# LahiruCooray/rl-aerial-manipulator

Hardware: AMD Instinct MI355X
Metric: env-steps/sec (whole node), hexacopter+arm waypoint task at 4096 envs/GPU (higher is better)
Workload: dtype f32

## Files before the change

rl-aerial-manipulator_amd/csrc/amenv_capi.hip:

```cpp
#include <hip/hip_runtime.h>
#include <hip/hip_ext.h>

#include <algorithm>
#include <cmath>
#include <cstdio>
#include <cstdlib>
#include <cstring>
#include <mutex>
#include <new>
#include <string>
#include <vector>

#include "amenv_kernels.hpp"
#include "amenv_team.hpp"
#include "amenv_team_host.hpp"
#include "amenv_quad.hpp"
#include "amenv_team_policy.hpp"
#include "amenv_quad_policy.hpp"
#include "amenv_lane_policy.hpp"
#include "amenv_rigid_policy.hpp"
#include "amenv_obsnorm.hpp"
#include "amenv_policy.hpp"
#include "amenv_train.hpp"
#include "amenv_mlp_train.hpp"
// ... 310 lines not shown
bool rigid_pol_ok(const amenv_config& c) { return c.vehicle.n_joints == 0 && c.dtype == AMENV_F32 && (c.vehicle.n_rotors == 4 || c.vehicle.n_rotors == 6); }
bool arm_pol_ok(const amenv_config& c) { return c.vehicle.n_joints == 3 && c.dtype == AMENV_F32; }

constexpr int kTeamAutoMax = 6144;
constexpr int kArmkAutoMax = 32768;

const char* select_step_family(const amenv_config& c, StepFamily* out) {
  const int want = c.step_kernel, n = c.num_envs;
  const bool autok = want == AMENV_KERNEL_AUTO, f32 = c.dtype == AMENV_F32, arm = zxx_arm1(c);
  StepFamily f = StepFamily::Lane;
  if (arm && (want == AMENV_KERNEL_TEAM || (f32 && autok && n <= kTeamAutoMax)))
    f = StepFamily::Team;
  else if (arm && c.task.rk4_substeps == 1 && (want == AMENV_KERNEL_STAGED || (f32 && autok && n > kTeamAutoMax && n <= kArmkAutoMax)))
    f = StepFamily::Staged;
  else if (arm && f32 && (want == AMENV_KERNEL_HELPER || (autok && n <= 65536)))
    f = StepFamily::TwoWave;
  else if (quad_ok(c) && want == AMENV_KERNEL_TEAM)
    f = StepFamily::Quad;
  else if (c.vehicle.n_joints == 0 && c.block_size == 0 && (autok ? n <= 32768 : want == AMENV_KERNEL_HELPER && n <= 64 * kStatsReplicas))
    f = StepFamily::LaneHelper;
  if (f == StepFamily::Lane && want == AMENV_KERNEL_HELPER)
    return "AMENV_KERNEL_HELPER is built for fp32 z,x,x-arm vehicles and for rigid vehicles with block_size = 0 "
           "and at most 65536 envs (its Monitor wave owns one of the 1024 replicas of the running totals per tile)";
  if (f == StepFamily::Lane && want == AMENV_KERNEL_TEAM)
    return "AMENV_KERNEL_TEAM is built for the 6-rotor vehicle with the z,x,x arm (16 lanes per env; fp64 = logic-gate build) and for "
           "fp32 rigid vehicles with 4 or 6 rotors, the single-waypoint v2 task and block_size = 0 (4 lanes per env)";
  if (f == StepFamily::Lane && want == AMENV_KERNEL_STAGED)
    return "AMENV_KERNEL_STAGED is built for the 6-rotor vehicle with the z,x,x arm (fp64 = logic-gate build), the single-waypoint v2 task "
           "and rk4_substeps = 1";
  *out = f;
  return nullptr;
}

std::string kernel_name(const amenv& e) {
  const amenv_config& c = e.cfg;
  const char* t = c.dtype == AMENV_F64 ? "double" : "float";
  const int nrot = (c.vehicle.n_rotors == 4 || c.vehicle.n_rotors == 6) ? c.vehicle.n_rotors : AMENV_MAX_ROTORS;
  const int kw = is_v1(&c) ? 2 : (c.task.num_waypoints == 1 ? 1 : AMENV_MAX_WAYPOINTS);
  char buf[200] = "";
  switch (e.family) {
    case StepFamily::Lane:
      std::snprintf(buf, sizeof(buf), "step_kernel<%s,NROT=%d,KW=%d,%s> block=%d", t, nrot, kw, c.vehicle.n_joints ? "v2+arm3" : (is_v1(&c) ? "v1" : "v2"), e.block); break;
    case StepFamily::LaneHelper:
      std::snprintf(buf, sizeof(buf), "step_kernel_pw<%s,NROT=%d,KW=%d,%s> (main wave + reset wave [+ observation wave + Monitor wave] per 64-env tile)", t, nrot, kw,
                    is_v1(&c) ? "v1" : "v2"); break;
    case StepFamily::Quad:
      std::snprintf(buf, sizeof(buf), "step_kernel_quad<NROT=%d,v2> (4 lanes per env, 16 envs per wave + episode-end helper wave)", c.vehicle.n_rotors); break;
    case StepFamily::Team:
      std::snprintf(buf, sizeof(buf), "step_kernel_team<%s,NROT=6,v2+arm3> (16 lanes per env: 4 RK4 stages x 4 components, 4 envs per wave + episode-end helper wave)", t); break;
    case StepFamily::Staged:
      std::snprintf(buf, sizeof(buf), "step_kernel_armk<%s,NROT=6> block=320 (4 RK4 stage waves + main wave per 64-env tile)", t); break;
    case StepFamily::TwoWave:
      std::snprintf(buf, sizeof(buf), "step_kernel_arm2w<float,NROT=6> block=128 (2 waves per 64-env tile)"); break;
  }
  std::string name = buf;
  if (e.dr) name += " +dr";
  if (e.pub_nj == 1 || e.pub_nj == 2) name += " [" + std::to_string(e.pub_nj) + "-joint arm: phantom links inside, pack / unpack at the C ABI]";
  return name;
}

template <typename... P, typename... A>
hipError_t launch(const amenv& e, bool timed, void (*k)(P...), dim3 grid, dim3 block, size_t lds, hipStream_t s, A... args) {
  if (timed) hipExtLaunchKernelGGL(k, grid, block, lds, s, e.ev_start, e.ev_stop, 0, args...);
  else hipLaunchKernelGGL(k, grid, block, lds, s, args...);
  return hipGetLastError();
}

template <typename T, int NROT, int KW, int VAR, int NJ, bool DR>
hipError_t launch_rollout(const amenv& e, const StepIO& io, int T_steps, hipStream_t s) {
  const StepTail tl{io.terminal_obs, io.ep_return, io.ep_len, io.stats};
  const ColdParams C = make_cold(e);
  const uint32_t tb = e.tile_bytes;
  const int32_t n = e.cfg.num_envs;
  switch (e.family) {
    case StepFamily::Team:
      if constexpr (NJ == 3 && sizeof(T) == 4 && !DR)
        return launch(e, false, rollout_kernel_team<NROT>, dim3(e.n_tiles * 16), dim3(64), 0, s, e.blob, tb, n, reinterpret_cast<const float*>(io.actions), io.obs,
                      static_cast<float*>(io.reward), io.done, io.info, T_steps, tl, C, make_team<T>(e));
      return hipErrorInvalidValue;
    case StepFamily::Quad:
      if constexpr (NJ == 0 && sizeof(T) == 4 && KW == 1 && VAR == VAR_V2 && (NROT == 4 || NROT == 6) && !DR)
        return launch(e, false, rollout_kernel_quad<NROT>, dim3(e.n_tiles * 4), dim3(64), 0, s, e.blob, tb, n, io.actions, io.obs, static_cast<float*>(io.reward), io.done,
                      io.info, T_steps, tl, C, make_quad(e));
      return hipErrorInvalidValue;
    case StepFamily::Lane: case StepFamily::LaneHelper: case StepFamily::Staged: case StepFamily::TwoWave:
      break;
  }
  ArmArg<T, NJ> AA;
  if constexpr (NJ > 0) AA.p = make_arm<T>(e); else AA.unused = 0;
  const int bs = e.block;
  return launch(e, false, rollout_kernel<T, NROT, KW, VAR, NJ, DR>, dim3((e.n_tiles * 64 + bs - 1) / bs), dim3(bs), size_t(bs) * ObsDim<VAR, NJ>::value * sizeof(float), s,
                e.blob, tb, n, io.actions, io.obs, io.reward, io.done, io.info, T_steps, tl, make_hot<T, NROT>(e), C, AA, make_dr<DR>(e));
}

template <typename T, int NROT, int KW, int VAR, int NJ = 0, bool DR = false>
hipError_t launch_step(const amenv& e, const StepIO& io, int T_steps, hipStream_t s, bool timed) {
  if (T_steps > 0) return launch_rollout<T, NROT, KW, VAR, NJ, DR>(e, io, T_steps, s);
  ArmArg<T, NJ> AA;
  if constexpr (NJ > 0) AA.p = make_arm<T>(e); else AA.unused = 0;
  const HotParams<T, NROT> P = make_hot<T, NROT>(e);
  const ColdParams C = make_cold(e);
  const StepTail tl{io.terminal_obs, io.ep_return, io.ep_len, io.stats};
  const uint32_t tb = e.tile_bytes;
  const int32_t n = e.cfg.num_envs;
  switch (e.family) {
    case StepFamily::Team:
      if constexpr (NJ == 3 && !DR) {
        const TeamParamsT<T> TP = make_team<T>(e);
        return launch(e, timed, step_kernel_team<T, NROT>, dim3(e.n_tiles * 16), dim3(128), 0, s, e.blob, n, int32_t(e.n_tiles * 16),
                      reinterpret_cast<const float*>(io.actions), TP.consts, io.obs, static_cast<T*>(io.reward), io.done, io.info, tl, C);
      }
      break;
    case StepFamily::Staged:
      if constexpr (NJ == 3 && !DR) {
        if constexpr (sizeof(T) == 8) {
          hipError_t ea = hipFuncSetAttribute(reinterpret_cast<const void*>(&step_kernel_armk<T, NROT>), hipFuncAttributeMaxDynamicSharedMemorySize, 96 * 1024);
          if (ea != hipSuccess) return ea;
        }
        const size_t lds = size_t(64 * ObsDim<VAR, NJ>::value + 12 * 64) * sizeof(float) + size_t((4 * kAggSlots + 6) * 64) * sizeof(T);
        return launch(e, timed, step_kernel_armk<T, NROT>, dim3(e.n_tiles), dim3(320), lds, s, e.blob, tb, n, io.actions, io.obs, io.reward, io.done, io.info, tl, P, C, AA);
      }
      break;
    case StepFamily::TwoWave:
      if constexpr (NJ == 3 && sizeof(T) == 4 && !DR) {
        const size_t lds = size_t(64 * ObsDim<VAR, NJ>::value + (kArmXchgSlots + 12) * 64) * sizeof(float);
        return launch(e, timed, step_kernel_arm2w<T, NROT>, dim3(e.n_tiles), dim3(128), lds, s, e.blob, tb, n, io.actions, io.obs, io.reward, io.done, io.info, tl, P, C, AA);
      }
      break;
    case StepFamily::Quad:
      if constexpr (NJ == 0 && sizeof(T) == 4 && KW == 1 && VAR == VAR_V2 && (NROT == 4 || NROT == 6) && !DR)
        return launch(e, timed, step_kernel_quad<NROT>, dim3(e.n_tiles * 4), dim3(128), 0, s, e.blob, tb, n, io.actions, io.obs, static_cast<float*>(io.reward), io.done,
                      io.info, tl, C, make_quad(e));
      break;
    case StepFamily::LaneHelper:
      if constexpr (NJ == 0) {
        const size_t lds = size_t(64 * ObsDim<VAR, 0>::value + 12 * 64) * sizeof(float);
        return launch(e, timed, step_kernel_pw<T, NROT, KW, VAR, DR>, dim3(e.n_tiles), dim3((KW == 1 && VAR == VAR_V2) ? 256 : 128), lds, s, e.blob, tb, n, io.actions,
                      io.obs, io.reward, io.done, io.info, tl, P, C, make_dr<DR>(e));
      }
      break;
    case StepFamily::Lane: {
      const int bs = e.block;
// ... 946 lines not shown
```

rl-aerial-manipulator_amd/csrc/amenv_team.hpp:

```cpp
#pragma once
#include "amenv_kernels.hpp"

#define AMENV_FN __device__ __forceinline__

namespace amenv_dev {

template <int CTRL> __device__ __forceinline__ float dpp_(float v) {
  return __builtin_bit_cast(float, __builtin_amdgcn_update_dpp(0, __builtin_bit_cast(int, v), CTRL, 0xF, 0xF, true));
}
template <int CTRL> __device__ __forceinline__ double dpp_(double v) {
  const int lo = __builtin_amdgcn_update_dpp(0, __double2loint(v), CTRL, 0xF, 0xF, true);
  const int hi = __builtin_amdgcn_update_dpp(0, __double2hiint(v), CTRL, 0xF, 0xF, true);
  return __hiloint2double(hi, lo);
}
template <int P0, int P1, int P2, int P3> __device__ __forceinline__ float qp(float v) { return dpp_<P0 | (P1 << 2) | (P2 << 4) | (P3 << 6)>(v); }
template <int P0, int P1, int P2, int P3> __device__ __forceinline__ double qp(double v) { return dpp_<P0 | (P1 << 2) | (P2 << 4) | (P3 << 6)>(v); }
template <int P0, int P1, int P2, int P3> __device__ __forceinline__ int qpi(int v) {
  return __builtin_amdgcn_update_dpp(0, v, P0 | (P1 << 2) | (P2 << 4) | (P3 << 6), 0xF, 0xF, true);
}
template <int N> __device__ __forceinline__ float row_ror(float v) { return dpp_<0x120 + N>(v); }
template <int N> __device__ __forceinline__ double row_ror(double v) { return dpp_<0x120 + N>(v); }
template <int N> __device__ __forceinline__ float row_shr(float v) { return dpp_<0x110 + N>(v); }
template <int N> __device__ __forceinline__ double row_shr(double v) { return dpp_<0x110 + N>(v); }
__device__ __forceinline__ float sel(bool m, float a, float b) { return m ? a : b; }
__device__ __forceinline__ double sel(bool m, double a, double b) { return m ? a : b; }
__device__ __forceinline__ int sel(bool m, int a, int b) { return m ? a : b; }
__device__ __forceinline__ void sincos_t(float x, float& s, float& c) { s = __sinf(x); c = __cosf(x); }
__device__ __forceinline__ void sincos_t(double x, double& s, double& c) { s = sin(x); c = cos(x); }
__device__ __forceinline__ float scale_action_f32(float a, float s1, float s2) { return (a * s1) * s2; }
__device__ __forceinline__ double scale_action_f32(double a, double s1, double s2) { return double((float(a) * float(s1)) * float(s2)); }
__device__ __forceinline__ float joint_cmd_f32(float a, float half, float mid) { return __builtin_fmaf(a, half, mid); }
__device__ __forceinline__ double joint_cmd_f32(double a, double half, double mid) { return double(__builtin_fmaf(float(a), float(half), float(mid))); }

}

#include "amenv_team_math.hpp"

namespace amenv_dev {

using TeamParams = TeamParamsT<float>;
using TeamState = TeamStateT<float>;

__device__ __forceinline__ int team_group_of_block(int b, int nblocks) { return (b & 7) * (nblocks >> 3) + (b >> 3); }

template <typename X>
struct TeamEnvT {
  TeamStateT<X> y;
  X WP;
  X final_yaw, last_distance, ep_return;
  int32_t step, counter, flags, episode;
};
using TeamEnv = TeamEnvT<float>;

template <typename X>
struct TeamLaneT {
  int lane, cc, bb;
  bool q0, q1, q2, lead;
  uint32_t offA, offB, offC;
  bool okA, okB, okC;
  X c[((kTeamConsts + 3) / 4) * 4];
  __device__ __forceinline__ void init(const TeamParamsT<X>& P) { init(P.consts); }
  __device__ __forceinline__ void init(const void* table) {
    lane = int(threadIdx.x) & 63; cc = lane & 3; bb = (lane >> 2) & 3;
    q0 = bb == 0; q1 = bb == 1; q2 = bb == 2; lead = (lane & 15) == 0;
    offA = uint32_t(cc + 3 * bb + (bb == 3 ? 1 : 0));
    offB = uint32_t(13 + 3 * bb - (bb == 3 ? 2 : 0) + (q2 ? 0 : cc));
    offC = uint32_t(23 + cc + (bb > 0 ? 3 : 0));
    okA = cc < 3 || q2; okB = q2 ? cc == 0 : cc < 3; okC = cc < 3 && bb < 2;
    constexpr int NC4 = (kTeamConsts + 3) / 4;
    if constexpr (sizeof(X) == 4) {
      const float4* tab = static_cast<const float4*>(table);
#pragma unroll
      for (int k = 0; k < NC4; k++) {
        const float4 v = tab[k * 16 + (lane & 15)];
        c[4 * k] = v.x; c[4 * k + 1] = v.y; c[4 * k + 2] = v.z; c[4 * k + 3] = v.w;
      }
// ... 20 lines not shown
__device__ __forceinline__ void team_load_unpack(TeamEnvT<X>& E) {
  E.final_yaw = bc<3>(E.y.P); E.last_distance = bc<3>(E.y.V); E.ep_return = bc<3>(E.y.W);
}
template <typename X>
__device__ __forceinline__ void team_load(const char* tile, int i, const TeamLaneT<X>& L, TeamEnvT<X>& E) {
  team_load_issue(tile, i, L, E);
  team_load_unpack(E);
}

template <typename X>
__device__ __forceinline__ void team_store(char* tile, int i, const TeamLaneT<X>& L, const TeamEnvT<X>& E, bool store_wp = true) {
  constexpr uint32_t GB = 64u * 4u * sizeof(X);
  const uint32_t eoff = (uint32_t(i & 63) * 4u + uint32_t(L.cc)) * uint32_t(sizeof(X));
  const bool l3 = L.cc == 3;
  const X g0 = sel(l3, E.final_yaw, E.y.P), g1 = sel(l3, E.last_distance, E.y.V), g3 = sel(l3, E.ep_return, E.y.W);
  const X sv = sel(L.q0, g0, sel(L.q1, g1, sel(L.q2, E.y.Q, g3)));
  *reinterpret_cast<X*>(tile + kIntBytes + uint32_t(L.bb) * GB + eoff) = sv;
  const int ival = sel(L.cc == 0, E.step, sel(L.cc == 1, E.counter, sel(L.cc == 2, E.flags, E.episode)));
  if constexpr (sizeof(X) == 4) {
    const float s2 = sel(L.q0, E.y.TH, sel(L.q1, E.y.THD, sel(L.q2, __int_as_float(ival), E.WP)));
    const uint32_t off2 = L.q2 ? eoff : kIntBytes + (L.q0 ? 5u : (L.q1 ? 6u : 4u)) * GB + eoff;
    if (L.q0 || L.q1 || L.q2 || store_wp) *reinterpret_cast<float*>(tile + off2) = s2;
  } else {
    if (L.q2) reinterpret_cast<int32_t*>(tile)[(i & 63) * 4 + L.cc] = ival;
    else if (L.q0 || L.q1 || store_wp) *reinterpret_cast<X*>(tile + kIntBytes + (L.q0 ? 5u : (L.q1 ? 6u : 4u)) * GB + eoff) = sel(L.q0, E.y.TH, sel(L.q1, E.y.THD, E.WP));
  }
}

template <typename X> struct TeamOutT { X reward; uint32_t bits; X vA, vB, vC; bool ended; int ep_len; float ep_ret; };
using TeamOut = TeamOutT<float>;

template <typename X> struct TeamResetT { X P, WP, final_yaw, vA, vB, vC; };
template <typename X>
__device__ __forceinline__ TeamResetT<X> team_reset(const TeamParamsT<X>& P, const ColdParams& C, const TeamLaneT<X>& L, int32_t episode, int i) {
  const X* c = L.c;
  uint32_t wds[4];
  const int64_t gid = C.gid0 + i;
  philox4x32_10(C.seed_lo, C.seed_hi, uint32_t(uint64_t(gid)), uint32_t(uint64_t(gid) >> 32), uint32_t(episode), uint32_t(L.cc), wds);
  uint32_t r[12];
#pragma unroll
  for (int k = 0; k < 4; k++) {
    r[k] = uint32_t(qpi<0, 0, 0, 0>(int(wds[k]))); r[4 + k] = uint32_t(qpi<1, 1, 1, 1>(int(wds[k]))); r[8 + k] = uint32_t(qpi<2, 2, 2, 2>(int(wds[k])));
  }
  Env<X, 1> e;
  e.episode = episode;
  reset_from_words<X, 1>(C, 1, e, r);
  const X e0 = c[TC_E0], e1 = c[TC_E1], e2 = c[TC_E2];
  TeamResetT<X> R;
  R.P = fma_(e0, e.px, fma_(e1, e.py, e2 * e.pz));
  R.WP = fma_(e0, e.wp[0][0], fma_(e1, e.wp[0][1], e2 * e.wp[0][2]));
  R.final_yaw = e.final_yaw;
  const X eo = fma_(e0, P.ee_home[0], fma_(e1, P.ee_home[1], e2 * P.ee_home[2]));
  const X zero = X(0), Q = L.cc == 0 ? X(1) : X(0);
  R.vA = (L.q0 ? R.P : (L.q1 ? zero : (L.q2 ? Q : zero))) * c[TC_OBS_A];
  const X tp = P.ee_task != 0 ? R.P + eo : R.P;
  R.vB = (L.q0 ? R.WP - tp : (L.q1 ? zero : (L.q2 ? R.final_yaw : zero))) * c[TC_OBS_B];
  R.vC = (L.q0 ? zero : eo) * c[TC_OBS_C];
  return R;
}

template <typename X>
__device__ __forceinline__ void team_apply_reset(const TeamLaneT<X>& L, const TeamResetT<X>& R, TeamEnvT<X>& E, TeamOutT<X>& o) {
  TeamStateT<X>& y = E.y;
  y.P = R.P; y.V = X(0); y.W = X(0); y.TH = X(0); y.THD = X(0);
  y.Q = L.cc == 0 ? X(1) : X(0);
  E.WP = R.WP; E.final_yaw = R.final_yaw;
  E.last_distance = X(-1); E.ep_return = X(0);
  E.step = 0; E.counter = 0; E.flags = 0; E.episode += 1;
  o.vA = R.vA; o.vB = R.vB; o.vC = R.vC;
  o.bits |= AMENV_INFO_WAS_RESET;
}

template <typename X>
__device__ __forceinline__ void team_obs_vals(const TeamParamsT<X>& P, const TeamLaneT<X>& L, const TeamEnvT<X>& E, X eo, X& vA, X& vB, X& vC) {
  const X* c = L.c;
  const TeamStateT<X>& z = E.y;
  vA = sel(L.q0, z.P, sel(L.q1, z.V, sel(L.q2, z.Q, z.W))) * c[TC_OBS_A];
  const X tp = P.ee_task != 0 ? z.P + eo : z.P;
  vB = sel(L.q0, E.WP - tp, sel(L.q1, X(0), sel(L.q2, E.final_yaw, z.TH))) * c[TC_OBS_B];
  vC = sel(L.q0, z.THD, eo) * c[TC_OBS_C];
}

template <int NROT, bool HELPED = false, typename X>
__device__ __forceinline__ TeamOutT<X> team_advance(const TeamParamsT<X>& P, const ColdParams& C, const TeamLaneT<X>& L, TeamEnvT<X>& E, X act, X actj, int i, bool active,
                                                    float* terminal_obs, float* ep_return_out, int32_t* ep_len_out) {
  constexpr int OD = 29;
  TeamStateT<X>& y = E.y;
#ifdef AMENV_TEAM_DIAG_NORK4
  const X EO = y.TH + act * actj;
#else
  const X EO = team_dynamics(P, L.c, L.q0, L.q1, L.q2, y, act, actj);
// ... 34 lines not shown
      }
      if (P.flags & AMENV_FLAG_AUTO_RESET) team_apply_reset(L, team_reset(P, C, L, E.episode, i), E, o);
    }
  }
  return o;
}

template <bool OPT, typename X>
__device__ __forceinline__ void team_store_outputs(const TeamLaneT<X>& L, const TeamOutT<X>& o, uint32_t i, bool active, float* __restrict__ obs, X* __restrict__ reward_out,
                                                   uint8_t* __restrict__ done, uint32_t* __restrict__ info) {
  const uint32_t row = i * 29u;
  const bool ob = active && (!OPT || obs != nullptr);
  if (ob && L.okA) obs[row + L.offA] = float(o.vA);
  if (ob && L.okB) obs[row + L.offB] = float(o.vB);
  if (ob && L.okC) obs[row + L.offC] = float(o.vC);
  if (active && L.lead) {
    if (!OPT || reward_out) reward_out[i] = o.reward;
    if (!OPT || done) done[i] = o.ended ? 1 : 0;
    if (!OPT || info) info[i] = o.bits;
  }
}

template <typename X> __device__ __forceinline__ void team_touch(X v) {
  if constexpr (sizeof(X) == 4) asm volatile("" ::"v"(v));
  else asm volatile("" ::"v"(__double2loint(v)), "v"(__double2hiint(v)));
}

template <typename A> __device__ __forceinline__ void team_arg(A a) { asm volatile("" ::"s"(a)); }
template <typename A, typename... R> __device__ __forceinline__ void team_arg(A a, R... r) { team_arg(a); team_arg(r...); }

__device__ __forceinline__ __amdgpu_buffer_rsrc_t team_rsrc(void* p, uint32_t bytes) { return __builtin_amdgcn_make_buffer_rsrc(p, 0, int(bytes), 0x00020000); }
constexpr uint32_t kOob = 0xFFFFFFFFu;

template <typename X, int NROT>
__global__ __launch_bounds__(128) void step_kernel_team(void* __restrict__ blob, int32_t n_envs, int32_t n_blocks, const float* __restrict__ actions,
                                                        const void* __restrict__ lane_consts, float* __restrict__ obs, X* __restrict__ reward_out,
                                                        uint8_t* __restrict__ done, uint32_t* __restrict__ info, const StepTail tl, const ColdParams C) {
  constexpr uint32_t tile_bytes = kIntBytes + 7u * 64u * 4u * uint32_t(sizeof(X));
  TeamParamsT<X> P;
  {
    typedef const __attribute__((address_space(4))) uint32_t ConstWord;
    ConstWord* src = (ConstWord*)(static_cast<const char*>(lane_consts) + team_table_bytes<X>());
    uint32_t* dst = reinterpret_cast<uint32_t*>(&P);
    static_assert(sizeof(TeamParamsT<X>) % 4 == 0, "copied word by word");
#pragma unroll
    for (int k = 0; k < int(sizeof(TeamParamsT<X>) / 4); k++) dst[k] = src[k];
  }
  static_assert(NROT == 6, "team kernel: 6-rotor airframe");
  constexpr int AD = 7, OD = 29;
  __shared__ X rst[6][64];
  __shared__ uint32_t fl[4][4];
  __shared__ uint32_t have[4];
  __shared__ unsigned long long acc[S_COUNT];
#ifdef AMENV_STAMPS
  unsigned long long stamps_[kStampSlots] = {0, 0, 0, 0, 0, 0, 0, 0};
#endif
  const int role = __builtin_amdgcn_readfirstlane(int(threadIdx.x) >> 6);
  team_arg(blob, n_envs, n_blocks, actions, lane_consts);
  AMENV_STAMP(0);
  TeamLaneT<X> L;
  L.init(lane_consts);
  const int row = L.lane >> 4;
  const int i0 = team_group_of_block(int(blockIdx.x), n_blocks) * 4;
  const int i = i0 + row;
  const bool active = i < n_envs;
  char* tile = static_cast<char*>(blob) + size_t(i0 >> 6) * tile_bytes;
  const int ia = active ? i : n_envs - 1;
  TeamEnvT<X> E;
  team_load_issue(tile, i, L, E);
  const float act_f = actions[size_t(ia) * AD + L.cc];
  const float actj_f = actions[size_t(ia) * AD + 4 + (L.cc < 3 ? L.cc : 2)];
#ifdef AMENV_TEAM_DIAG_NOHELPER
  if (role == 1) { __syncthreads(); return; }
#endif
  if (role == 1) {
#pragma unroll
    for (int k = 0; k < kTeamConsts; k++)
      if (k < TC_ALLOC0 || k >= TC_GV1) team_touch(L.c[k]);
    team_touch(E.y.Q); team_touch(E.y.W); team_touch(E.y.TH); team_touch(E.y.THD); team_touch(E.WP); team_touch(act_f); team_touch(actj_f);
    const bool owned = n_blocks <= kStatsReplicas;
    if (L.lane < S_COUNT) acc[L.lane] = 0ull;
    const X dtc = P.h * X(P.substeps), slack = X(0.01) + X(50) * dtc * dtc;
    const X reach = fma_(dtc, abs_(E.y.V), abs_(E.y.P)) + slack;
    const bool lane_may = (L.cc < 3 && !(reach < X(5.7735))) || (L.cc == 2 && !(E.y.P - dtc * abs_(E.y.V) - slack > X(0.1)));
    const unsigned long long mm = __ballot(lane_may);
#ifdef AMENV_TEAM_DIAG_NOPREDICT
    constexpr bool kPredict = false;
#else
    constexpr bool kPredict = true;
#endif
    const bool may = kPredict && (((mm >> (L.lane & 48)) & 0xFFFFull) != 0ull || E.step >= P.max_steps || ((E.flags & AMENV_FLAGBIT_FWR) && E.counter >= P.counter_limit) ||
                                  (P.flags & AMENV_FLAG_NAN_GUARD));
    if (L.lead) have[row] = may ? 1u : 0u;
    unsigned long long* totals = tl.stats + size_t(blockIdx.x & (kStatsReplicas - 1)) * kStatsStride;
    unsigned long long mine = 0ull;
    bool fetched = false;
    if (__ballot(may) != 0ull) {
      if (owned && L.lane < S_COUNT) mine = totals[L.lane];
      fetched = true;
      if (may) {
        const TeamResetT<X> R = team_reset(P, C, L, E.episode, i);
        rst[0][L.lane] = R.P; rst[1][L.lane] = R.WP; rst[2][L.lane] = R.final_yaw;
        rst[3][L.lane] = R.vA; rst[4][L.lane] = R.vB; rst[5][L.lane] = R.vC;
      }
    }
    __syncthreads();
#ifdef AMENV_TEAM_DIAG_NOPOST
    return;
#endif
    const bool ended = (fl[row][0] & 1u) != 0 && L.lead;
    if (__ballot(ended) != 0ull) {
      if (!fetched && owned && L.lane < S_COUNT) mine = totals[L.lane];
      if (ended) {
        const uint32_t bits = fl[row][1];
        const int ep_len = int(fl[row][2]);
        const float ep_ret = __uint_as_float(fl[row][3]);
        if (tl.ep_return) tl.ep_return[i] = ep_ret;
        if (tl.ep_len) tl.ep_len[i] = ep_len;
        if (owned) accumulate_stats_lane(acc, 0, bits, ep_len, ep_ret);
        else accumulate_stats_lane(tl.stats, int(blockIdx.x), bits, ep_len, ep_ret);
      }
      if (owned) {
        __builtin_amdgcn_fence(__ATOMIC_ACQ_REL, "wavefront");
        __builtin_amdgcn_wave_barrier();
        if (L.lane < S_COUNT) totals[L.lane] = mine + acc[L.lane];
      }
    }
    return;
  }
#ifndef AMENV_TEAM_DIAG_NOPRIO
  __builtin_amdgcn_s_setprio(3);
#endif
  team_load_unpack(E);
  const X act = X(act_f), actj = X(actj_f);
  const uint32_t obs_bytes = uint32_t(n_envs) * uint32_t(OD * 4);
  const uint32_t rowb = uint32_t(i) * uint32_t(OD * 4);
  uint32_t voA = L.okA ? rowb + L.offA * 4u : kOob, voB = L.okB ? rowb + L.offB * 4u : kOob, voC = L.okC ? rowb + L.offC * 4u : kOob;
  asm volatile("" : "+v"(voA), "+v"(voB), "+v"(voC));
  const __amdgpu_buffer_rsrc_t r_obs = team_rsrc(obs, obs_bytes), r_term = team_rsrc(tl.terminal_obs, tl.terminal_obs ? obs_bytes : 0u);
  AMENV_STAMP(1);
  AMENV_STAMP_DRAIN();
  AMENV_STAMP(2);
  TeamOutT<X> o = team_advance<NROT, true>(P, C, L, E, act, actj, i, active, nullptr, nullptr, nullptr);
  const bool resets = o.ended && (P.flags & AMENV_FLAG_AUTO_RESET);
  if (L.lead) {
    fl[row][0] = (o.ended && active ? 1u : 0u) | (resets ? 2u : 0u);
    if (o.ended) { fl[row][1] = o.bits; fl[row][2] = uint32_t(o.ep_len); fl[row][3] = __float_as_uint(o.ep_ret); }
  }
  AMENV_STAMP(4);
#ifdef AMENV_STAMPS
  stamps_[3] = __ballot(o.ended && active) != 0ull ? 1ull : 0ull;
#endif
  __syncthreads();
  const bool any_end = __ballot(o.ended) != 0ull;
  const X tA = o.vA, tB = o.vB, tC = o.vC;
  if (any_end && resets) {
    TeamResetT<X> R;
    if (have[row]) R = TeamResetT<X>{rst[0][L.lane], rst[1][L.lane], rst[2][L.lane], rst[3][L.lane], rst[4][L.lane], rst[5][L.lane]};
    else R = team_reset(P, C, L, E.episode, i);
    team_apply_reset(L, R, E, o);
  }
  AMENV_STAMP(5);
  team_store(tile, i, L, E, resets);
  __builtin_amdgcn_raw_buffer_store_b32(__float_as_int(float(o.vA)), r_obs, int(voA), 0, 0);
  __builtin_amdgcn_raw_buffer_store_b32(__float_as_int(float(o.vB)), r_obs, int(voB), 0, 0);
  __builtin_amdgcn_raw_buffer_store_b32(__float_as_int(float(o.vC)), r_obs, int(voC), 0, 0);
  if (active && L.lead) { reward_out[uint32_t(i)] = o.reward; done[uint32_t(i)] = o.ended ? 1 : 0; info[uint32_t(i)] = o.bits; }
  if (any_end) {
    __builtin_amdgcn_raw_buffer_store_b32(__float_as_int(float(tA)), r_term, int(o.ended ? voA : kOob), 0, 0);
    __builtin_amdgcn_raw_buffer_store_b32(__float_as_int(float(tB)), r_term, int(o.ended ? voB : kOob), 0, 0);
    __builtin_amdgcn_raw_buffer_store_b32(__float_as_int(float(tC)), r_term, int(o.ended ? voC : kOob), 0, 0);
  }
  AMENV_STAMP(6);
#ifdef AMENV_STAMPS
  AMENV_STAMP_DRAIN();
  AMENV_STAMP(7);
  if (L.lane == 0 && blockIdx.x < kStampWaves)
    for (int kk = 0; kk < kStampSlots; kk++) tl.stats[kStampBase + blockIdx.x * kStampSlots + kk] = stamps_[kk];
#endif
}

template <int NROT>
__global__ __launch_bounds__(64) void rollout_kernel_team(void* __restrict__ blob, uint32_t tile_bytes, int32_t n_envs, const float* __restrict__ actions,
                                                          float* __restrict__ obs, float* __restrict__ reward_out, uint8_t* __restrict__ done,
                                                          uint32_t* __restrict__ info, int n_steps, const StepTail tl, const ColdParams C, const TeamParams P) {
  constexpr int AD = 7, OD = 29;
  TeamLane L;
  L.init(P);
  const int i = team_group_of_block(int(blockIdx.x), int(gridDim.x)) * 4 + (L.lane >> 4);
  const bool active = i < n_envs;
  const int ia = active ? i : n_envs - 1;
  char* tile = static_cast<char*>(blob) + size_t(i >> 6) * tile_bytes;
  TeamEnv E;
  team_load(tile, i, L, E);
  const size_t n = size_t(n_envs);
  const uint32_t ja = uint32_t(L.cc < 3 ? L.cc : 2);
  const float* ap = actions + size_t(ia) * AD;
  float act = ap[L.cc], actj = ap[4 + ja];
  for (int t = 0; t < n_steps; t++) {
    const float a_now = act, aj_now = actj;
    if (t + 1 < n_steps) { ap += n * AD; act = ap[L.cc]; actj = ap[4 + ja]; }
    const TeamOut o = team_advance<NROT>(P, C, L, E, a_now, aj_now, i, active, nullptr, nullptr, nullptr);
    accumulate_stats(tl.stats, int(blockIdx.x), o.bits, active && o.ended && L.lead, o.ep_len, o.ep_ret);
    const size_t tn = size_t(t) * n;
    team_store_outputs<true>(L, o, uint32_t(i), active, obs ? obs + tn * OD : nullptr, reward_out ? reward_out + tn : nullptr, done ? done + tn : nullptr,
                       info ? info + tn : nullptr);
  }
  team_store(tile, i, L, E);
}

}
// ... 1 lines not shown
```

rl-aerial-manipulator_amd/csrc/amenv_team_math.hpp:

```cpp
#pragma once
#include <stddef.h>
#include <stdint.h>

namespace amenv_dev {

template <typename X> struct LaneTraits { using T = X; using M = bool; };

enum TeamConst {
  TC_E0 = 0, TC_E1, TC_E2, TC_GV,
  TC_SP, TC_SQ, TC_SR, TC_O0,
  TC_ACT1, TC_ACT2, TC_JHALF, TC_JMID,
  TC_ALLOC0, TC_MIX0 = TC_ALLOC0 + 6,
  TC_GV1 = TC_MIX0 + 6, TC_GV2,
  TC_E01, TC_ZX,
  TC_I0C0, TC_I0C1, TC_I0C2,
  TC_I1C0, TC_I1C1, TC_I1C2,
  TC_LC0, TC_O1,
  TC_NTR0, TC_NTR_END = TC_NTR0 + 9,
  TC_ALC0 = TC_NTR_END, TC_ALC1, TC_ALC2, TC_ALC3,
  TC_TMIN, TC_TMAX,
  TC_MXQ0, TC_MXQ1, TC_MXQ2, TC_MXQ3,
  TC_OBS_A, TC_OBS_B, TC_OBS_C,
  TC_HSTEP,
  TC_WGT,
// ... 35 lines not shown
template <typename X> struct TM { X c0, c1, c2; };
template <typename X> AMENV_FN X matvec(const TM<X>& M, X v) { return fma_(M.c0, bc<0>(v), fma_(M.c1, bc<1>(v), M.c2 * bc<2>(v))); }

template <int AX, typename X>
AMENV_FN void rotate_cols(TM<X>& R, X s, X co) {
  X& a = AX == 0 ? R.c1 : (AX == 1 ? R.c2 : R.c0);
  X& b = AX == 0 ? R.c2 : (AX == 1 ? R.c0 : R.c1);
  const X ra = a, rb = b;
  a = fma_(co, ra, s * rb);
  b = fma_(co, rb, -(s * ra));
}

template <typename X, typename PT> AMENV_FN X joint_accel(const PT& P, X cmd, X th, X thd) {
  return clamp_(fma_(P.kp, cmd - th, -(P.kd * thd)), -P.amax, P.amax);
}

template <typename X> struct TeamStage {
  X3<X> S, U;
  X Aa;
  TM<X> Ic, C, L;
  X c0;
};

template <typename X, typename PT>
AMENV_FN TeamStage<X> team_kin_stage(const PT& P, const X* c, X TH, X THD, X thdd, X Fe2, X Mv) {
  using T = typename LaneTraits<X>::T;
  const X e0 = c[TC_E0], e1 = c[TC_E1], e2 = c[TC_E2];
  X S, U, Aa, Tn;
  TM<X> IO{c[TC_I0C0], c[TC_I0C1], c[TC_I0C2]};
  TM<X> G{T(0), T(0), T(0)};
  X sIO = T(0), sG = T(0);
  TM<X> R;
  X p, pd, pdd, w, al;
  {
    X s, co;
    sincos_t(bc<0>(TH), s, co);
    const X td = bc<0>(THD), tdd = bc<0>(thdd);
    const X cov = fma_(co, c[TC_E01], e2), sv = s * c[TC_ZX];
    auto zrot = [&](X v) { return fma_(cov, v, sv * qp<1, 0, 2, 3>(v)); };
    auto zx = [&](X v) { return c[TC_ZX] * qp<1, 0, 2, 3>(v); };
    R.c0 = fma_(co, e0, s * e1); R.c1 = fma_(co, e1, -(s * e0)); R.c2 = e2;
    p = c[TC_O0];
    {
      const T m = P.lm[0];
      const X Rc = zrot(c[TC_LC0]), zRc = zx(Rc);
      const X r = p + Rc, u = td * zRc;
      const X a_ = fma_(tdd, zRc, td * zx(u));
      const X A0 = zrot(c[TC_I1C0]), A1 = zrot(c[TC_I1C1]), A2 = zrot(c[TC_I1C2]);
      const TM<X> J{fma_(co, A0, -(s * A1)), fma_(s, A0, co * A1), A2};
      S = m * r; U = m * u; Aa = m * a_;
      const X mr = m * r;
      sIO = m * dot3(r, r);
      const X r0 = bc<0>(r), r1 = bc<1>(r), r2 = bc<2>(r);
      IO.c0 = IO.c0 + fma_(-mr, r0, J.c0); IO.c1 = IO.c1 + fma_(-mr, r1, J.c1); IO.c2 = IO.c2 + fma_(-mr, r2, J.c2);
      const T m2 = m + m;
      const X mu = m2 * u;
      sG = m2 * dot3(u, r);
      G.c0 = fma_(td, zx(fma_(T(2), J.c0, c[TC_NTR0 + 0])), -(mu * r0));
      G.c1 = fma_(td, zx(fma_(T(2), J.c1, c[TC_NTR0 + 1])), -(mu * r1));
      G.c2 = fma_(td, zx(fma_(T(2), J.c2, c[TC_NTR0 + 2])), -(mu * r2));
      Tn = fma_(m, cross_c(x3(r), a_), fma_(tdd, J.c2, (td * td) * zx(J.c2)));
    }
    {
      X s2, co2;
      sincos_t(bc<1>(TH), s2, co2);
      const X td1 = bc<1>(THD), tdd1 = bc<1>(thdd);
      const X Ro = zrot(c[TC_O1]), zRo = zx(Ro);
      pd = td * zRo;
      pdd = fma_(tdd, zRo, td * zx(pd));
      p = p + Ro;
      const X z = R.c0;
      al = fma_(td1, td * zx(z), fma_(tdd1, z, tdd * e2));
      w = fma_(td1, z, td * e2);
      rotate_cols<0>(R, s2, co2);
    }
  }
  auto link = [&](int k) {
    const T m = P.lm[k];
    const X Rc = fma_(R.c0, P.lcm[k][0], fma_(R.c1, P.lcm[k][1], R.c2 * P.lcm[k][2]));
    const X3<X> xw = x3(w), xRc = x3(Rc);
    const X wRc = cross(xw, xRc);
    const X r = p + Rc, u = pd + wRc;
    const X a_ = pdd + cross_c(xw, wRc) - cross_c(xRc, al);
    const X RI0 = fma_(R.c0, P.li[k][0], fma_(R.c1, P.li[k][1], R.c2 * P.li[k][2]));
    const X RI1 = fma_(R.c0, P.li[k][1], fma_(R.c1, P.li[k][3], R.c2 * P.li[k][4]));
    const X RI2 = fma_(R.c0, P.li[k][2], fma_(R.c1, P.li[k][4], R.c2 * P.li[k][5]));
    const TM<X> J{fma_(RI0, bc<0>(R.c0), fma_(RI1, bc<0>(R.c1), RI2 * bc<0>(R.c2))), fma_(RI0, bc<1>(R.c0), fma_(RI1, bc<1>(R.c1), RI2 * bc<1>(R.c2))),
                  fma_(RI0, bc<2>(R.c0), fma_(RI1, bc<2>(R.c1), RI2 * bc<2>(R.c2)))};
    S = fma_(m, r, S); U = fma_(m, u, U); Aa = fma_(m, a_, Aa);
    const X mr = m * r;
    sIO = fma_(m, dot3(r, r), sIO);
    const X r0 = bc<0>(r), r1 = bc<1>(r), r2 = bc<2>(r);
    IO.c0 = IO.c0 + fma_(-mr, r0, J.c0); IO.c1 = IO.c1 + fma_(-mr, r1, J.c1); IO.c2 = IO.c2 + fma_(-mr, r2, J.c2);
    const T m2 = m + m;
    const X mu = m2 * u;
    sG = fma_(m2, dot3(u, r), sG);
    G.c0 = G.c0 + (cross_c(xw, fma_(T(2), J.c0, c[TC_NTR0 + 3 * k + 0])) - mu * r0);
    G.c1 = G.c1 + (cross_c(xw, fma_(T(2), J.c1, c[TC_NTR0 + 3 * k + 1])) - mu * r1);
    G.c2 = G.c2 + (cross_c(xw, fma_(T(2), J.c2, c[TC_NTR0 + 3 * k + 2])) - mu * r2);
    const X Jw = matvec(J, w);
    Tn = Tn + (fma_(m, cross_c(x3(r), a_), matvec(J, al)) + cross_c(xw, Jw));
  };
  auto advance_x = [&](X th, X td, X tdd, const T* o) {
    X s, co;
    sincos_t(th, s, co);
    const X Ro = fma_(R.c0, o[0], fma_(R.c1, o[1], R.c2 * o[2]));
    const X3<X> xRo = x3(Ro), xw = x3(w);
    const X wRo = cross(xw, xRo);
    pd = pd + wRo;
    pdd = pdd + (cross_c(xw, wRo) - cross_c(xRo, al));
    p = p + Ro;
    const X z = R.c0;
    const X wz = cross_c(xw, z);
    al = fma_(td, wz, fma_(tdd, z, al));
    w = fma_(td, z, w);
    rotate_cols<0>(R, s, co);
  };
  link(1);
  advance_x(bc<2>(TH), bc<2>(THD), bc<2>(thdd), P.o2);
  link(2);
  TeamStage<X> k;
  const T im = P.inv_mtot;
  const X imS2 = im * dot3(S, S), imS = im * S;
  const X S0 = bc<0>(S), S1 = bc<1>(S), S2 = bc<2>(S);
  const X dI = sIO - imS2;
  k.Ic = TM<X>{fma_(imS, S0, fma_(dI, e0, IO.c0)), fma_(imS, S1, fma_(dI, e1, IO.c1)), fma_(imS, S2, fma_(dI, e2, IO.c2))};
  const X3<X> x0 = x3(k.Ic.c0), x1 = x3(k.Ic.c1), x2 = x3(k.Ic.c2);
  const TM<X> A{cross(x1, x2), cross(x2, x0), cross(x0, x1)};
  const X idet = rcp_(dot3(x0.v, A.c0));
  k.C = TM<X>{idet * A.c0, idet * A.c1, idet * A.c2};
  const T im2 = im + im;
  const X imU2 = im2 * U, dL = fma_(im2, dot3(S, U), -sG);
  k.L = TM<X>{fma_(-imU2, S0, fma_(dL, e0, -G.c0)), fma_(-imU2, S1, fma_(dL, e1, -G.c1)), fma_(-imU2, S2, fma_(dL, e2, -G.c2))};
  k.S = x3(S); k.U = x3(U); k.Aa = Aa;
  k.c0 = fma_(im, cross_c(k.S, Aa - Fe2), Mv - Tn);
  return k;
}

template <typename X> AMENV_FN X team_wdot(const TeamStage<X>& k, X W) {
  const X b0 = bc<0>(W), b1 = bc<1>(W), b2 = bc<2>(W);
  const X IcW = fma_(k.Ic.c0, b0, fma_(k.Ic.c1, b1, k.Ic.c2 * b2));
  const X LW = fma_(k.L.c0, b0, fma_(k.L.c1, b1, fma_(k.L.c2, b2, k.c0)));
  return matvec(k.C, LW - cross_c(x3(W), IcW));
}
template <typename X> AMENV_FN X team_qdot(const X* c, X Q, X W) {
  using T = typename LaneTraits<X>::T;
  const X n2 = sum4(Q * Q);
  X dq = fma_(T(-2), n2, T(2)) * Q;
  dq = fma_(c[TC_SP] * bc<0>(W), qp<1, 0, 3, 2>(Q), dq);
  dq = fma_(c[TC_SQ] * bc<1>(W), qp<2, 3, 0, 1>(Q), dq);
  dq = fma_(c[TC_SR] * bc<2>(W), qp<3, 2, 1, 0>(Q), dq);
  return dq;
}
template <typename X, typename PT> AMENV_FN X team_vdot(const PT& P, const X* c, const TeamStage<X>& k, X Q, X W, X wd, X Fe2) {
  using T = typename LaneTraits<X>::T;
  const X n2 = sum4(Q * Q);
  const X two_in2 = T(2) * rcp_(n2);
  const X3<X> qv{qp<1, 2, 3, 3>(Q), qp<2, 3, 1, 3>(Q), qp<3, 1, 2, 3>(Q)};
  const X qw = bc<0>(Q);
  const X3<X> om = x3(W);
  const X3<X> gv{c[TC_GV], c[TC_GV1], c[TC_GV2]};
  const X gb = fma_(two_in2, cross_c(qv, fma_(qw, gv.v, cross(qv, gv))), gv.v);
  const X fb = fma_(T(2), cross(om, k.U), cross_c(om, cross(om, k.S))) + k.Aa;
  const X f = Fe2 + fma_(P.mtot, gb, -fb);
  const X Aacc = P.inv_mtot * (f + cross_c(k.S, wd));
  return fma_(two_in2, cross_c(qv, fma_(-qw, Aacc, cross_c(qv, Aacc))), Aacc);
}

template <typename X, typename PT> AMENV_FN X team_tool_offset(const PT& P, const X* c, const TeamStateT<X>& y) {
  using T = typename LaneTraits<X>::T;
  const X e0 = c[TC_E0], e1 = c[TC_E1], e2 = c[TC_E2];
  X s, co;
  sincos_t(bc<0>(y.TH), s, co);
  TM<X> R{fma_(co, e0, s * e1), fma_(co, e1, -(s * e0)), e2};
  X p = c[TC_O0];
  p = p + fma_(R.c0, P.o1[0], fma_(R.c1, P.o1[1], R.c2 * P.o1[2]));
  sincos_t(bc<1>(y.TH), s, co);
  rotate_cols<0>(R, s, co);
  p = p + fma_(R.c0, P.o2[0], fma_(R.c1, P.o2[1], R.c2 * P.o2[2]));
  sincos_t(bc<2>(y.TH), s, co);
  rotate_cols<0>(R, s, co);
  p = p + fma_(R.c0, P.tool[0], fma_(R.c1, P.tool[1], R.c2 * P.tool[2]));
  const X3<X> qv{qp<1, 2, 3, 3>(y.Q), qp<2, 3, 1, 3>(y.Q), qp<3, 1, 2, 3>(y.Q)};
  const X qw = bc<0>(y.Q);
  return fma_(T(2), cross_c(qv, fma_(-qw, p, cross_c(qv, p))), p);
}

template <typename X> struct TeamStageDeriv { X dV, dQ, dW, Qs, Ws; };

template <typename X, typename PT, typename M>
AMENV_FN X team_dynamics(const PT& P, const X* c, M q0, M q1, M q2, TeamStateT<X>& y, X act, X actj, TeamStageDeriv<X>* probe = nullptr) {
  using T = typename LaneTraits<X>::T;
  const X uu = scale_action_f32(act, c[TC_ACT1], c[TC_ACT2]);
  X t = fma_(c[TC_ALC0], bc<0>(uu), fma_(c[TC_ALC1], bc<1>(uu), fma_(c[TC_ALC2], bc<2>(uu), c[TC_ALC3] * bc<3>(uu))));
  t = clamp_(t, c[TC_TMIN], c[TC_TMAX]);
  const X wr = sum_bodies(fma_(c[TC_MXQ0], bc<0>(t), fma_(c[TC_MXQ1], bc<1>(t), fma_(c[TC_MXQ2], bc<2>(t), c[TC_MXQ3] * bc<3>(t)))));
  const X Fe2 = bc<0>(wr) * c[TC_E2], Mv = qp<1, 2, 3, 3>(wr);
  const X cmd = joint_cmd_f32(actj, c[TC_JHALF], c[TC_JMID]);
  const T h = P.h, hh = T(0.5) * h, h6 = h * T(1.0 / 6.0);
  const X hs = c[TC_HSTEP], wgt = c[TC_WGT], pw = c[TC_PW];
  int it = 0;
  do {
    const X a1 = joint_accel(P, cmd, y.TH, y.THD);
    const X TH2 = fma_(hh, y.THD, y.TH), THD2 = fma_(hh, a1, y.THD), a2 = joint_accel(P, cmd, TH2, THD2);
    const X TH3 = fma_(hh, THD2, y.TH), THD3 = fma_(hh, a2, y.THD), a3 = joint_accel(P, cmd, TH3, THD3);
    const X TH4 = fma_(h, THD3, y.TH), THD4 = fma_(h, a3, y.THD), a4 = joint_accel(P, cmd, TH4, THD4);
    const X THs = sel(q0, y.TH, sel(q1, TH2, sel(q2, TH3, TH4))), THDs = sel(q0, y.THD, sel(q1, THD2, sel(q2, THD3, THD4)));
    const X as = sel(q0, a1, sel(q1, a2, sel(q2, a3, a4)));
    const TeamStage<X> k = team_kin_stage(P, c, THs, THDs, as, Fe2, Mv);
    X Wc = y.W, Qc = y.Q, wd, dq;
#pragma unroll
    for (int s = 0; s < 4; s++) {
      wd = team_wdot(k, Wc);
// ... 19 lines not shown
```

Measured before the change: 885.6 million.

## Share one episode-end helper wave across four integrating waves in team kernel

When the grid is small relative to the CU count, the team kernel launches 320-thread blocks in which four integrating waves share one helper wave, instead of one helper per integrating wave. The helper now precomputes only the random reset draw, and each lane builds its reset observation itself. The change also computes the three joint sincos values in one lane-parallel call instead of three serial calls, and uses buffer stores with out-of-range offsets for the tile, reward, done and info writes so the stores need no branches. The aim is to cut helper-wave overhead and sincos cost, at the price of larger blocks and a new grid mapping that only applies when there are few tiles.

```diff
diff --git a/rl-aerial-manipulator_amd/csrc/amenv_capi.hip b/rl-aerial-manipulator_amd/csrc/amenv_capi.hip
--- a/rl-aerial-manipulator_amd/csrc/amenv_capi.hip
+++ b/rl-aerial-manipulator_amd/csrc/amenv_capi.hip
@@ -366,6 +366,18 @@
   return nullptr;
 }
 
+static bool team_wide(const amenv& e) {
+  static std::mutex m;
+  static int cus[64] = {0};
+  const int d = e.device >= 0 && e.device < 64 ? e.device : 0;
+  std::lock_guard<std::mutex> g(m);
+  if (cus[d] == 0) {
+    int v = 0;
+    cus[d] = hipDeviceGetAttribute(&v, hipDeviceAttributeMultiprocessorCount, d) == hipSuccess && v > 0 ? v : 1;
+  }
+  return e.n_tiles * 4 <= cus[d];
+}
+
 std::string kernel_name(const amenv& e) {
   const amenv_config& c = e.cfg;
   const char* t = c.dtype == AMENV_F64 ? "double" : "float";
@@ -381,7 +393,8 @@
     case StepFamily::Quad:
       std::snprintf(buf, sizeof(buf), "step_kernel_quad<NROT=%d,v2> (4 lanes per env, 16 envs per wave + episode-end helper wave)", c.vehicle.n_rotors); break;
     case StepFamily::Team:
-      std::snprintf(buf, sizeof(buf), "step_kernel_team<%s,NROT=6,v2+arm3> (16 lanes per env: 4 RK4 stages x 4 components, 4 envs per wave + episode-end helper wave)", t); break;
+      std::snprintf(buf, sizeof(buf), "step_kernel_team<%s,NROT=6,v2+arm3> (16 lanes per env: 4 RK4 stages x 4 components, 4 envs per wave + %s)", t,
+                    team_wide(e) ? "one episode-end helper wave per 4" : "episode-end helper wave"); break;
     case StepFamily::Staged:
       std::snprintf(buf, sizeof(buf), "step_kernel_armk<%s,NROT=6> block=320 (4 RK4 stage waves + main wave per 64-env tile)", t); break;
     case StepFamily::TwoWave:
@@ -441,7 +454,10 @@
     case StepFamily::Team:
       if constexpr (NJ == 3 && !DR) {
         const TeamParamsT<T> TP = make_team<T>(e);
-        return launch(e, timed, step_kernel_team<T, NROT>, dim3(e.n_tiles * 16), dim3(128), 0, s, e.blob, n, int32_t(e.n_tiles * 16),
+        if (team_wide(e))
+          return launch(e, timed, step_kernel_team<T, NROT, 4>, dim3(e.n_tiles * 4), dim3(320), 0, s, e.blob, n, int32_t(e.n_tiles * 4),
+                        reinterpret_cast<const float*>(io.actions), TP.consts, io.obs, static_cast<T*>(io.reward), io.done, io.info, tl, C);
+        return launch(e, timed, step_kernel_team<T, NROT, 1>, dim3(e.n_tiles * 16), dim3(128), 0, s, e.blob, n, int32_t(e.n_tiles * 16),
                       reinterpret_cast<const float*>(io.actions), TP.consts, io.obs, static_cast<T*>(io.reward), io.done, io.info, tl, C);
       }
       break;
diff --git a/rl-aerial-manipulator_amd/csrc/amenv_team.hpp b/rl-aerial-manipulator_amd/csrc/amenv_team.hpp
--- a/rl-aerial-manipulator_amd/csrc/amenv_team.hpp
+++ b/rl-aerial-manipulator_amd/csrc/amenv_team.hpp
@@ -42,6 +42,8 @@
 using TeamState = TeamStateT<float>;
 
 __device__ __forceinline__ int team_group_of_block(int b, int nblocks) { return (b & 7) * (nblocks >> 3) + (b >> 3); }
+
+__device__ __forceinline__ int team_group16_of_block(int b, int nblocks) { return (nblocks & 7) ? b : (b & 7) * (nblocks >> 3) + (b >> 3); }
 
 template <typename X>
 struct TeamEnvT {
@@ -128,11 +130,10 @@
 
 template <typename X> struct TeamResetT { X P, WP, final_yaw, vA, vB, vC; };
 template <typename X>
-__device__ __forceinline__ TeamResetT<X> team_reset(const TeamParamsT<X>& P, const ColdParams& C, const TeamLaneT<X>& L, int32_t episode, int i) {
-  const X* c = L.c;
+__device__ __forceinline__ TeamResetT<X> team_reset_draw(const ColdParams& C, const X* c, int cc, int32_t episode, int i) {
   uint32_t wds[4];
   const int64_t gid = C.gid0 + i;
-  philox4x32_10(C.seed_lo, C.seed_hi, uint32_t(uint64_t(gid)), uint32_t(uint64_t(gid) >> 32), uint32_t(episode), uint32_t(L.cc), wds);
+  philox4x32_10(C.seed_lo, C.seed_hi, uint32_t(uint64_t(gid)), uint32_t(uint64_t(gid) >> 32), uint32_t(episode), uint32_t(cc), wds);
   uint32_t r[12];
 #pragma unroll
   for (int k = 0; k < 4; k++) {
@@ -146,6 +147,13 @@
   R.P = fma_(e0, e.px, fma_(e1, e.py, e2 * e.pz));
   R.WP = fma_(e0, e.wp[0][0], fma_(e1, e.wp[0][1], e2 * e.wp[0][2]));
   R.final_yaw = e.final_yaw;
+  R.vA = R.vB = R.vC = X(0);
+  return R;
+}
+template <typename X>
+__device__ __forceinline__ TeamResetT<X> team_reset_obs(const TeamParamsT<X>& P, const TeamLaneT<X>& L, TeamResetT<X> R) {
+  const X* c = L.c;
+  const X e0 = c[TC_E0], e1 = c[TC_E1], e2 = c[TC_E2];
   const X eo = fma_(e0, P.ee_home[0], fma_(e1, P.ee_home[1], e2 * P.ee_home[2]));
   const X zero = X(0), Q = L.cc == 0 ? X(1) : X(0);
   R.vA = (L.q0 ? R.P : (L.q1 ? zero : (L.q2 ? Q : zero))) * c[TC_OBS_A];
@@ -153,6 +161,10 @@
   R.vB = (L.q0 ? R.WP - tp : (L.q1 ? zero : (L.q2 ? R.final_yaw : zero))) * c[TC_OBS_B];
   R.vC = (L.q0 ? zero : eo) * c[TC_OBS_C];
   return R;
+}
+template <typename X>
+__device__ __forceinline__ TeamResetT<X> team_reset(const TeamParamsT<X>& P, const ColdParams& C, const TeamLaneT<X>& L, int32_t episode, int i) {
+  return team_reset_obs(P, L, team_reset_draw<X>(C, L.c, L.cc, episode, i));
 }
 
 template <typename X>
@@ -253,8 +265,8 @@
 __device__ __forceinline__ __amdgpu_buffer_rsrc_t team_rsrc(void* p, uint32_t bytes) { return __builtin_amdgcn_make_buffer_rsrc(p, 0, int(bytes), 0x00020000); }
 constexpr uint32_t kOob = 0xFFFFFFFFu;
 
-template <typename X, int NROT>
-__global__ __launch_bounds__(128) void step_kernel_team(void* __restrict__ blob, int32_t n_envs, int32_t n_blocks, const float* __restrict__ actions,
+template <typename X, int NROT, int MW>
+__global__ __launch_bounds__(64 * (MW + 1)) void step_kernel_team(void* __restrict__ blob, int32_t n_envs, int32_t n_blocks, const float* __restrict__ actions,
                                                         const void* __restrict__ lane_consts, float* __restrict__ obs, X* __restrict__ reward_out,
                                                         uint8_t* __restrict__ done, uint32_t* __restrict__ info, const StepTail tl, const ColdParams C) {
   constexpr uint32_t tile_bytes = kIntBytes + 7u * 64u * 4u * uint32_t(sizeof(X));
@@ -269,20 +281,23 @@
   }
   static_assert(NROT == 6, "team kernel: 6-rotor airframe");
   constexpr int AD = 7, OD = 29;
-  __shared__ X rst[6][64];
-  __shared__ uint32_t fl[4][4];
-  __shared__ uint32_t have[4];
+  __shared__ X rst[3][64];
+  static_assert(MW == 1 || MW == 4, "one helper wave of 64 lanes = 16 quads serves at most four integrating waves");
+  constexpr int ROWS = 4 * MW;
+  __shared__ uint32_t fl[ROWS][4];
+  __shared__ uint32_t have[ROWS];
   __shared__ unsigned long long acc[S_COUNT];
 #ifdef AMENV_STAMPS
   unsigned long long stamps_[kStampSlots] = {0, 0, 0, 0, 0, 0, 0, 0};
 #endif
-  const int role = __builtin_amdgcn_readfirstlane(int(threadIdx.x) >> 6);
+  const int wave = __builtin_amdgcn_readfirstlane(int(threadIdx.x) >> 6);
+  const int role = wave == MW ? 1 : 0;
   team_arg(blob, n_envs, n_blocks, actions, lane_consts);
   AMENV_STAMP(0);
   TeamLaneT<X> L;
   L.init(lane_consts);
-  const int row = L.lane >> 4;
-  const int i0 = team_group_of_block(int(blockIdx.x), n_blocks) * 4;
+  const int row = role ? L.lane >> 2 : wave * 4 + (L.lane >> 4);
+  const int i0 = (MW == 1 ? team_group_of_block(int(blockIdx.x), n_blocks) : team_group16_of_block(int(blockIdx.x), n_blocks)) * ROWS;
   const int i = i0 + row;
   const bool active = i < n_envs;
   char* tile = static_cast<char*>(blob) + size_t(i0 >> 6) * tile_bytes;
@@ -310,9 +325,11 @@
 #else
     constexpr bool kPredict = true;
 #endif
-    const bool may = kPredict && (((mm >> (L.lane & 48)) & 0xFFFFull) != 0ull || E.step >= P.max_steps || ((E.flags & AMENV_FLAGBIT_FWR) && E.counter >= P.counter_limit) ||
+    const bool serve = row < ROWS;
+    const bool hlead = serve && L.cc == 0;
+    const bool may = kPredict && serve && (((mm >> (L.lane & 60)) & 0xFull) != 0ull || E.step >= P.max_steps || ((E.flags & AMENV_FLAGBIT_FWR) && E.counter >= P.counter_limit) ||
                                   (P.flags & AMENV_FLAG_NAN_GUARD));
-    if (L.lead) have[row] = may ? 1u : 0u;
+    if (hlead) have[row] = may ? 1u : 0u;
     unsigned long long* totals = tl.stats + size_t(blockIdx.x & (kStatsReplicas - 1)) * kStatsStride;
     unsigned long long mine = 0ull;
     bool fetched = false;
@@ -320,16 +337,15 @@
       if (owned && L.lane < S_COUNT) mine = totals[L.lane];
       fetched = true;
       if (may) {
-        const TeamResetT<X> R = team_reset(P, C, L, E.episode, i);
+        const TeamResetT<X> R = team_reset_draw<X>(C, L.c, L.cc, E.episode, i);
         rst[0][L.lane] = R.P; rst[1][L.lane] = R.WP; rst[2][L.lane] = R.final_yaw;
-        rst[3][L.lane] = R.vA; rst[4][L.lane] = R.vB; rst[5][L.lane] = R.vC;
       }
     }
     __syncthreads();
 #ifdef AMENV_TEAM_DIAG_NOPOST
     return;
 #endif
-    const bool ended = (fl[row][0] & 1u) != 0 && L.lead;
+    const bool ended = hlead && (fl[hlead ? row : 0][0] & 1u) != 0;
     if (__ballot(ended) != 0ull) {
       if (!fetched && owned && L.lane < S_COUNT) mine = totals[L.lane];
       if (ended) {
@@ -359,6 +375,15 @@
   uint32_t voA = L.okA ? rowb + L.offA * 4u : kOob, voB = L.okB ? rowb + L.offB * 4u : kOob, voC = L.okC ? rowb + L.offC * 4u : kOob;
   asm volatile("" : "+v"(voA), "+v"(voB), "+v"(voC));
   const __amdgpu_buffer_rsrc_t r_obs = team_rsrc(obs, obs_bytes), r_term = team_rsrc(tl.terminal_obs, tl.terminal_obs ? obs_bytes : 0u);
+  uint32_t so1 = 0, so2 = 0, voR = kOob, voD = kOob;
+  if constexpr (sizeof(X) == 4) {
+    constexpr uint32_t GB = 64u * 4u * 4u;
+    const uint32_t eoff = (uint32_t(i & 63) * 4u + uint32_t(L.cc)) * 4u;
+    so1 = kIntBytes + uint32_t(L.bb) * GB + eoff;
+    so2 = L.q2 ? eoff : kIntBytes + (L.q0 ? 5u : (L.q1 ? 6u : 4u)) * GB + eoff;
+    voR = active && L.lead ? uint32_t(i) * 4u : kOob; voD = active && L.lead ? uint32_t(i) : kOob;
+    asm volatile("" : "+v"(so1), "+v"(so2), "+v"(voR), "+v"(voD));
+  }
   AMENV_STAMP(1);
   AMENV_STAMP_DRAIN();
   AMENV_STAMP(2);
@@ -377,16 +402,35 @@
   const X tA = o.vA, tB = o.vB, tC = o.vC;
   if (any_end && resets) {
     TeamResetT<X> R;
-    if (have[row]) R = TeamResetT<X>{rst[0][L.lane], rst[1][L.lane], rst[2][L.lane], rst[3][L.lane], rst[4][L.lane], rst[5][L.lane]};
-    else R = team_reset(P, C, L, E.episode, i);
-    team_apply_reset(L, R, E, o);
+    const int hl = row * 4 + L.cc;
+    if (have[row]) R = TeamResetT<X>{rst[0][hl], rst[1][hl], rst[2][hl], X(0), X(0), X(0)};
+    else R = team_reset_draw<X>(C, L.c, L.cc, E.episode, i);
+    team_apply_reset(L, team_reset_obs(P, L, R), E, o);
   }
   AMENV_STAMP(5);
-  team_store(tile, i, L, E, resets);
+  if constexpr (sizeof(X) == 4) {
+    const __amdgpu_buffer_rsrc_t r_tile = team_rsrc(tile, tile_bytes);
+    const bool l3 = L.cc == 3;
+    const X g0 = sel(l3, E.final_yaw, E.y.P), g1 = sel(l3, E.last_distance, E.y.V), g3 = sel(l3, E.ep_return, E.y.W);
+    const X sv = sel(L.q0, g0, sel(L.q1, g1, sel(L.q2, E.y.Q, g3)));
+    __builtin_amdgcn_raw_buffer_store_b32(__float_as_int(sv), r_tile, int(so1), 0, 0);
+    const int ival = sel(L.cc == 0, E.step, sel(L.cc == 1, E.counter, sel(L.cc == 2, E.flags, E.episode)));
+    const float s2 = sel(L.q0, E.y.TH, sel(L.q1, E.y.THD, sel(L.q2, __int_as_float(ival), E.WP)));
+    __builtin_amdgcn_raw_buffer_store_b32(__float_as_int(s2), r_tile, int(L.bb == 3 && !resets ? kOob : so2), 0, 0);
+  } else {
+    team_store(tile, i, L, E, resets);
+  }
   __builtin_amdgcn_raw_buffer_store_b32(__float_as_int(float(o.vA)), r_obs, int(voA), 0, 0);
   __builtin_amdgcn_raw_buffer_store_b32(__float_as_int(float(o.vB)), r_obs, int(voB), 0, 0);
   __builtin_amdgcn_raw_buffer_store_b32(__float_as_int(float(o.vC)), r_obs, int(voC), 0, 0);
-  if (active && L.lead) { reward_out[uint32_t(i)] = o.reward; done[uint32_t(i)] = o.ended ? 1 : 0; info[uint32_t(i)] = o.bits; }
+  if constexpr (sizeof(X) == 4) {
+    const uint32_t nb = uint32_t(n_envs);
+    __builtin_amdgcn_raw_buffer_store_b32(__float_as_int(o.reward), team_rsrc(reward_out, nb * 4u), int(voR), 0, 0);
+    __builtin_amdgcn_raw_buffer_store_b8(uint8_t(o.ended ? 1 : 0), team_rsrc(done, nb), int(voD), 0, 0);
+    __builtin_amdgcn_raw_buffer_store_b32(int(o.bits), team_rsrc(info, nb * 4u), int(voR), 0, 0);
+  } else {
+    if (active && L.lead) { reward_out[uint32_t(i)] = o.reward; done[uint32_t(i)] = o.ended ? 1 : 0; info[uint32_t(i)] = o.bits; }
+  }
   if (any_end) {
     __builtin_amdgcn_raw_buffer_store_b32(__float_as_int(float(tA)), r_term, int(o.ended ? voA : kOob), 0, 0);
     __builtin_amdgcn_raw_buffer_store_b32(__float_as_int(float(tB)), r_term, int(o.ended ? voB : kOob), 0, 0);
@@ -396,8 +440,8 @@
 #ifdef AMENV_STAMPS
   AMENV_STAMP_DRAIN();
   AMENV_STAMP(7);
-  if (L.lane == 0 && blockIdx.x < kStampWaves)
-    for (int kk = 0; kk < kStampSlots; kk++) tl.stats[kStampBase + blockIdx.x * kStampSlots + kk] = stamps_[kk];
+  if (L.lane == 0 && blockIdx.x * MW + wave < kStampWaves)
+    for (int kk = 0; kk < kStampSlots; kk++) tl.stats[kStampBase + (blockIdx.x * MW + wave) * kStampSlots + kk] = stamps_[kk];
 #endif
 }
 
diff --git a/rl-aerial-manipulator_amd/csrc/amenv_team_math.hpp b/rl-aerial-manipulator_amd/csrc/amenv_team_math.hpp
--- a/rl-aerial-manipulator_amd/csrc/amenv_team_math.hpp
+++ b/rl-aerial-manipulator_amd/csrc/amenv_team_math.hpp
@@ -91,9 +91,10 @@
   X sIO = T(0), sG = T(0);
   TM<X> R;
   X p, pd, pdd, w, al;
+  X sT, cT;
+  sincos_t(TH, sT, cT);
   {
-    X s, co;
-    sincos_t(bc<0>(TH), s, co);
+    const X s = bc<0>(sT), co = bc<0>(cT);
     const X td = bc<0>(THD), tdd = bc<0>(thdd);
     const X cov = fma_(co, c[TC_E01], e2), sv = s * c[TC_ZX];
     auto zrot = [&](X v) { return fma_(cov, v, sv * qp<1, 0, 2, 3>(v)); };
@@ -121,8 +122,7 @@
       Tn = fma_(m, cross_c(x3(r), a_), fma_(tdd, J.c2, (td * td) * zx(J.c2)));
     }
     {
-      X s2, co2;
-      sincos_t(bc<1>(TH), s2, co2);
+      const X s2 = bc<1>(sT), co2 = bc<1>(cT);
       const X td1 = bc<1>(THD), tdd1 = bc<1>(thdd);
       const X Ro = zrot(c[TC_O1]), zRo = zx(Ro);
       pd = td * zRo;
@@ -160,9 +160,7 @@
     const X Jw = matvec(J, w);
     Tn = Tn + (fma_(m, cross_c(x3(r), a_), matvec(J, al)) + cross_c(xw, Jw));
   };
-  auto advance_x = [&](X th, X td, X tdd, const T* o) {
-    X s, co;
-    sincos_t(th, s, co);
+  auto advance_x = [&](X s, X co, X td, X tdd, const T* o) {
     const X Ro = fma_(R.c0, o[0], fma_(R.c1, o[1], R.c2 * o[2]));
     const X3<X> xRo = x3(Ro), xw = x3(w);
     const X wRo = cross(xw, xRo);
@@ -176,7 +174,7 @@
     rotate_cols<0>(R, s, co);
   };
   link(1);
-  advance_x(bc<2>(TH), bc<2>(THD), bc<2>(thdd), P.o2);
+  advance_x(bc<2>(sT), bc<2>(cT), bc<2>(THD), bc<2>(thdd), P.o2);
   link(2);
   TeamStage<X> k;
   const T im = P.inv_mtot;
@@ -229,15 +227,16 @@
 template <typename X, typename PT> AMENV_FN X team_tool_offset(const PT& P, const X* c, const TeamStateT<X>& y) {
   using T = typename LaneTraits<X>::T;
   const X e0 = c[TC_E0], e1 = c[TC_E1], e2 = c[TC_E2];
-  X s, co;
-  sincos_t(bc<0>(y.TH), s, co);
+  X sT, cT;
+  sincos_t(y.TH, sT, cT);
+  X s = bc<0>(sT), co = bc<0>(cT);
   TM<X> R{fma_(co, e0, s * e1), fma_(co, e1, -(s * e0)), e2};
   X p = c[TC_O0];
   p = p + fma_(R.c0, P.o1[0], fma_(R.c1, P.o1[1], R.c2 * P.o1[2]));
-  sincos_t(bc<1>(y.TH), s, co);
+  s = bc<1>(sT); co = bc<1>(cT);
   rotate_cols<0>(R, s, co);
   p = p + fma_(R.c0, P.o2[0], fma_(R.c1, P.o2[1], R.c2 * P.o2[2]));
-  sincos_t(bc<2>(y.TH), s, co);
+  s = bc<2>(sT); co = bc<2>(cT);
   rotate_cols<0>(R, s, co);
   p = p + fma_(R.c0, P.tool[0], fma_(R.c1, P.tool[1], R.c2 * P.tool[2]));
   const X3<X> qv{qp<1, 2, 3, 3>(y.Q), qp<2, 3, 1, 3>(y.Q), qp<3, 1, 2, 3>(y.Q)};
```

Result: faster. 935.1 million, median of 6 (+5.6%).
